# itxtx/normalizing-flows-study

Hardware: AMD Instinct MI355X
Metric: log_prob samples/sec/GPU + test-NLL match; RealNVP d=2 and MAF d=63 (higher is better)
Workload: dtype fp32

## Files before the change

include/nfx.h:

```cpp
#ifndef NFX_H
#define NFX_H

#include <stddef.h>
#include <stdint.h>

#ifdef __cplusplus
extern "C" {
#endif

#define NFX_ABI_VERSION 3

#define NFX_OK 0
#define NFX_EINVAL (-1)
#define NFX_EUNSUPPORTED (-2)
#define NFX_ELAUNCH (-3)

#define NFX_FORWARD 1
#define NFX_INVERSE (-1)

#define NFX_MAF_INVERSE 0
#define NFX_IAF_FORWARD 1
#define NFX_MAF_FORWARD 2
#define NFX_IAF_INVERSE 3

// ... 73 lines not shown
                          int64_t N, int K, float min_bin_width, float min_bin_height, float min_derivative,
                          int inverse, void* stream);

size_t nfx_arqs_packed_floats(int d, int H, int K);
int nfx_arqs_pack(const NfxMlpRaw* made, int d, int H, int K, float* packed, void* stream);
int nfx_arqs(const float* packed, const float* in, float* out, float* log_det, int64_t B, int d,
             int H, int K, float min_bin_width, float min_bin_height, float min_derivative,
             int rescale, double data_min, double data_max, int direction, int accumulate,
             void* stream);

int nfx_base_normal(uint64_t seed, uint64_t* rng_state, float* z, int64_t B, int d, void* stream);

size_t nfx_made_packed_floats(int d, int H);
int nfx_made_pack(const NfxMlpRaw* net, int d, int H, float* packed, void* stream);
int nfx_made_pack_parallel(const NfxMlpRaw* net, int d, int H, float* packed, void* stream);
int nfx_made_pack_sequential(int d, int H, float* packed, void* stream);
int nfx_made_affine(const float* packed, const float* in, float* out, float* log_det,
                    int64_t B, int d, int H, int variant, int accumulate, void* stream);
#define NFX_MADE_SEQ_AUTO 0
#define NFX_MADE_SEQ_SEGMENT 1
#define NFX_MADE_SEQ_WAVE 2
#define NFX_MADE_SEQ_PUSH 3
int nfx_made_seq_policy(int policy);
int nfx_made_affine_logprob(const float* packed, const float* in, float* out, float* log_det,
                            float* logp, double* sums, void* workspace, int64_t B, int d, int H,
                            int variant, int accumulate, void* stream);
int nfx_made_sample_supported(int d, int H, int variant);
int nfx_made_affine_sample(const float* packed, uint64_t seed, uint64_t* rng_state, float* z, float* x,
                           float* log_det, int64_t B, int d, int H, void* stream);

int nfx_made_pack_backward(const NfxMlpRaw* net, int d, int H, float* packed, void* stream);
size_t nfx_made_backward_factor_floats(int64_t B, int d, int H);
int64_t nfx_made_backward_max_batch(int d, int H);
int nfx_made_affine_backward(const float* packed, const float* in, const float* grad_out,
                             const float* grad_log_det, float* grad_in, float* factors, int64_t B,
                             int d, int H, int variant, void* stream);

int nfx_made_seq_backward(const float* packed, const float* in, const float* grad_out,
                          const float* grad_log_det, float* grad_in, float* factors, int64_t B,
                          int d, int H, int variant, void* stream);
int64_t nfx_made_factor_pitch(int64_t B);
size_t nfx_made_param_floats(int d, int H);
size_t nfx_made_wgrad_workspace_bytes(int64_t B, int d, int H);
int nfx_made_backward_weights(const float* factors, int64_t B, int d, int H,
                              const float* const* masks, float* grads, void* workspace,
                              void* stream);
// ... 247 lines not shown
```

normalizing-flows-study_amd/csrc/nfx_made.hip:

```cpp
#include "nfx_made_kernel.h"
#include "nfx_made_wide_kernel.h"
#include <atomic>
#include <cstdlib>

#include "nfx_made_seqs_kernel.h"
#include "nfx_pack.h"

namespace nfx {

__global__ void made_pack_kernel(NfxMlpRaw net, int d, int H, float* packed) {
    const int HT = (H + 31) / 32;
    const MadeLayout L = made_layout(d, HT);
    const int Hp = L.Hp, G1 = 4 * L.NKC;
    for (int i = blockIdx.x * blockDim.x + threadIdx.x; i < L.total; i += gridDim.x * blockDim.x) {
        if (i >= L.s_deg) continue;
        float v = 0.f;
        if (i < L.b1) {
            int t = i - L.w1, rr = t & 3, lane = (t >> 2) & 63, g = (t >> 8) % G1, ht = (t >> 8) / G1;
            int row = 32 * ht + (lane & 31), col = 2 * (4 * g + rr) + (lane >> 5);
            v = (row < H && col < d) ? mlp_weight(net, 0, d, row, col) : 0.f;
        } else if (i < L.w2) {
            int row = acc_vec_row(i - L.b1);
            v = row < H ? mlp_bias(net, 0, row) : 0.f;
        } else if (i < L.b2 || (i >= L.w3 && i < L.b3)) {
            const int layer = i < L.b2 ? 1 : 2;
            const ATileElem e = a_tile_elem(i - (layer == 1 ? L.w2 : L.w3));
            int row = 32 * (e.tile / HT) + e.row, col = 32 * (e.tile % HT) + e.k;
            v = (row < H && col < H) ? mlp_weight(net, layer, H, row, col) : 0.f;
        } else if (i < L.w3 || (i >= L.b3 && i < L.w4)) {
            const int layer = i < L.w3 ? 1 : 2;
            int row = acc_vec_row(i - (layer == 1 ? L.b2 : L.b3));
            v = row < H ? mlp_bias(net, layer, row) : 0.f;
        } else if (i < L.b4) {
            const ATileElem e = a_tile_elem(i - L.w4);
            int jw = e.tile / HT, which = jw & 1, j = jw >> 1;
            int orow = 32 * j + e.row, col = 32 * (e.tile % HT) + e.k;
            v = (orow < d && col < H) ? mlp_weight(net, 3, H, which * d + orow, col) : 0.f;
        } else if (i < L.par_total) {
            int t = i - L.b4, jw = t >> 5, which = jw & 1, j = jw >> 1;
            int orow = 32 * j + acc_vec_row(t & 31);
// ... 37 lines not shown
            if (a < H && net.mask[0]) {
                const float* row = net.mask[0] + (size_t)a * d;
#pragma unroll 4
                for (int j = q; j < d; j += 16) n += row[j] != 0.f ? 1 : 0;
            }
            n += __shfl_xor(n, 1);
            n += __shfl_xor(n, 2);
            n += __shfl_xor(n, 4);
            n += __shfl_xor(n, 8);
            if (q == 0 && a < Hp) deg[a] = a < H ? (net.mask[0] ? n - 1 : 0) : 1000000000;
        }
        __syncthreads();
        for (int a = threadIdx.x; a < Hp; a += kLiveThreads) {
            const int da = deg[a];
            int rank = 0;
            for (int b = 0; b < Hp; ++b) rank += (deg[b] < da || (deg[b] == da && b < a)) ? 1 : 0;
            packed[L.s_deg + a] = (float)da;
            packed[L.s_deg + Hp + rank] = (float)da;
            packed[L.s_deg + 2 * Hp + rank] = (float)a;
        }
    }
    int* nk = reinterpret_cast<int*>(packed);
    for (int i = threadIdx.x; i < 3 * HT + L.NJ; i += kLiveThreads) nk[L.nk1 + i] = 0;
    __shared__ double red[256];
    const int rows[4] = {H, H, H, 2 * d}, cols[4] = {d, H, H, H};
    const double tsafe = block_mlp_tsafe(net, 4, rows, cols, 1.0e37, red);
    if (threadIdx.x == 0) packed[L.tsafe] = (float)fmin(tsafe, 3.0e38);
}

__global__ __launch_bounds__(256) void made_extent_kernel(int d, int H, float* packed) {
    const int HT = (H + 31) / 32;
    const MadeLayout L = made_layout(d, HT);
    int* nk = reinterpret_cast<int*>(packed);
    const int n1 = HT * 4 * L.NKC, n23 = HT * HT * 4, n4 = L.NJ * 2 * HT * 4;
    const int lane = lane_id();
    for (int gi = blockIdx.x * 4 + (threadIdx.x >> 6); gi < n1 + 2 * n23 + n4; gi += gridDim.x * 4) {
        int off, word, ext;
        if (gi < n1) {
            const int ht = gi / (4 * L.NKC), g = gi % (4 * L.NKC);
            off = L.w1 + gi * 256;
            word = L.nk1 + ht;
            ext = g / 4 + 1;
        } else if (gi < n1 + 2 * n23) {
            const int t = (gi - n1) % n23, layer = (gi - n1) / n23;
            off = (layer == 0 ? L.w2 : L.w3) + t * 256;
            word = (layer == 0 ? L.nk2 : L.nk3) + t / (HT * 4);
            ext = (t % (HT * 4)) / 4 + 1;
        } else {
            const int t = gi - n1 - 2 * n23;
            off = L.w4 + t * 256;
            word = L.nk4 + t / (2 * HT * 4);
            ext = (t % (HT * 4)) / 4 + 1;
        }
        const f32x4 v = *reinterpret_cast<const f32x4*>(packed + off + 4 * lane);
        const bool nzl = v[0] != 0.f || v[1] != 0.f || v[2] != 0.f || v[3] != 0.f;
        if (__ballot(nzl) != 0 && lane == 0) atomicMax(&nk[word], ext);
    }
}

template <int HT>
made_seqs_kernel_t made_seqs_pick_ht(int variant, bool logp) {
// ... 60 lines not shown
    return made_pack_seqp(d, H, packed, s);
}
}

extern "C" int nfx_made_pack_parallel(const NfxMlpRaw* net, int d, int H, float* packed, void* stream) {
    if (!net || !packed) return set_error(NFX_EINVAL, "made_pack: null pointer");
    if (d <= 0 || d > 4096 || H <= 0 || H > 256)
        return set_error(NFX_EUNSUPPORTED, "made_pack: d=%d H=%d outside d<=4096, H<=256", d, H);
    if (net->n_layers != 4) return set_error(NFX_EINVAL, "made_pack: MADE has 4 masked layers (got %d)", net->n_layers);
    for (int l = 0; l < 4; ++l)
        if (!net->w[l]) return set_error(NFX_EINVAL, "made_pack: layer %d weight is null", l);
    const int total = (int)nfx_made_packed_floats(d, H);
    int blocks = (total + 255) / 256;
    if (blocks > 2048) blocks = 2048;
    made_pack_kernel<<<blocks, 256, 0, (hipStream_t)stream>>>(*net, d, H, packed);
    int rc = check_launch("made_pack_kernel");
    if (rc) return rc;
    made_live_kernel<<<1, kLiveThreads, 0, (hipStream_t)stream>>>(*net, d, H, packed);
    rc = check_launch("made_live_kernel");
    if (rc) return rc;
    {
        const int HT = (H + 31) / 32;
        const MadeLayout L = made_layout(d, HT);
        const int groups = HT * 4 * L.NKC + 2 * HT * HT * 4 + L.NJ * 2 * HT * 4;
        made_extent_kernel<<<(groups + 3) / 4, 256, 0, (hipStream_t)stream>>>(d, H, packed);
    }
    return check_launch("made_extent_kernel");
}

extern "C" int nfx_made_pack_sequential(int d, int H, float* packed, void* stream) {
    if (!packed) return set_error(NFX_EINVAL, "made_pack_sequential: null pointer");
    if (d <= 0 || d > 4096 || H <= 0 || H > 256)
        return set_error(NFX_EUNSUPPORTED, "made_pack_sequential: d=%d H=%d outside d<=4096, H<=256", d, H);
    return made_pack_seq(d, H, packed, (hipStream_t)stream);
}

extern "C" int nfx_made_pack(const NfxMlpRaw* net, int d, int H, float* packed, void* stream) {
    const int rc = nfx_made_pack_parallel(net, d, H, packed, stream);
    if (rc) return rc;
    return made_pack_seq(d, H, packed, (hipStream_t)stream);
}

namespace nfx {
int made_seqw_launch(const float* packed, const float* in, float* out, float* log_det, int64_t B, int d, int H,
                     int variant, int accumulate, float* logp, double* partials, double* sums, bool fused,
                     int* grid_out, hipStream_t s);
int made_seqp_launch(const float* packed, const float* in, float* out, float* log_det, int64_t B, int d, int H,
                     int variant, int accumulate, float* logp, double* partials, double* sums, bool fused,
                     hipStream_t s);
}

static std::atomic<int>& made_seq_policy() {
    static std::atomic<int> v{[] {
        const char* e = getenv("NFX_MADE_SEQ_POLICY");
        return e ? atoi(e) : NFX_MADE_SEQ_AUTO;
    }()};
    return v;
}

namespace nfx {
int made_seq_policy_get() { return made_seq_policy().load(std::memory_order_relaxed); }
}

static bool tile_path(int d, int HT, int variant) {
    return (variant == NFX_MAF_INVERSE || variant == NFX_IAF_FORWARD) && d > 0 && d <= kTileMaxD && HT >= 1 && HT <= 4;
}

struct TileConfig {
    int nw;
    bool wlds;
    size_t lds;
};
static TileConfig tile_config(const MadeLayout& L, int64_t ntiles, bool fused) {
    int nw = 8;
    if (!fused && ntiles < 4 * (int64_t)num_cus()) nw = (int)((ntiles + num_cus() - 1) / num_cus());
    const size_t wbytes = (size_t)L.par_total * sizeof(float);
    const size_t tiles = nw * 32 * (size_t)kTileStride * sizeof(float);
    const bool wlds = nw == 8 && wbytes + tiles <= kLdsBytes;
    return {nw, wlds, (wlds ? wbytes : 0) + tiles};
}

static int made_launch(const float* packed, const float* in, float* out, float* log_det, int64_t B,
                       int d, int H, int variant, int accumulate, float* logp, double* sums,
                       void* workspace, hipStream_t s) {
// ... 20 lines not shown
                         "made_affine_logprob: fused log_prob needs MAF inverse with d <= %d or H <= 64, "
                         "or IAF inverse with H <= 64", kTileMaxD);
    if (fused && B > 0 && (!logp || !workspace)) return set_error(NFX_EINVAL, "made_affine_logprob: null logp/workspace");
    if (B == 0) return fused ? gauss_finish(reinterpret_cast<double*>(workspace), 0, sums, 0, s) : NFX_OK;
    if (!packed || !in || !out || !log_det) return set_error(NFX_EINVAL, "made_affine: null pointer");
    if (in == out) return set_error(NFX_EINVAL, "made_affine: in and out must not alias");
    double* partials = reinterpret_cast<double*>(workspace);
    if (wide) {
        const int64_t nchunks = (B + 63) / 64;
        const int nw = nchunks < (int64_t)kWideWaves * num_cus() ? 4 : kWideWaves;
        const size_t lds_nw = (size_t)wide_lds(L, HT, nw).total * sizeof(float);
        made_par_kernel_t k = HT == 1 ? made_wide_pick_ht<1>(variant, fused, nw) : made_wide_pick_ht<2>(variant, fused, nw);
        int rc = prepare_lds((const void*)k, lds_nw);
        if (rc) return rc;
        int grid = resident_grid((const void*)k, 64 * nw, lds_nw, (nchunks + nw - 1) / nw);
        if (grid > kMaxPartials) grid = kMaxPartials;
        k<<<grid, 64 * nw, lds_nw, s>>>(packed, in, out, log_det, B, d, accumulate, nchunks, logp, partials,
                                        sums, gauss_const(d));
        return check_launch("made_wide_kernel");
    }
    if (tile_path(d, HT, variant)) {
        const int64_t ntiles = (B + 31) / 32;
        const TileConfig c = tile_config(L, ntiles, fused);
        made_par_kernel_t k = pick_tile(HT, c.wlds, variant, fused);
        if (!k) return set_error(NFX_EUNSUPPORTED, "made_affine: no kernel for H=%d", H);
        int rc = prepare_lds((const void*)k, c.lds);
        if (rc) return rc;
        int grid = resident_grid((const void*)k, 64 * c.nw, c.lds, (ntiles + c.nw - 1) / c.nw);
        if (grid > kMaxPartials) grid = kMaxPartials;
        k<<<grid, 64 * c.nw, c.lds, s>>>(packed, in, out, log_det, B, d, accumulate, ntiles, logp, partials, sums,
                                         gauss_const(d));
        return check_launch("made_tile_kernel");
    }
    if (variant == NFX_MAF_INVERSE || variant == NFX_IAF_FORWARD) {
        const size_t wbytes = (size_t)L.par_total * sizeof(float);
        const size_t stage8 = 8 * (size_t)kStageFloats * sizeof(float);
        const bool wlds = wbytes + stage8 <= kLdsBytes;
        made_par_kernel_t k = pick_par(HT, wlds, variant);
        if (!k) return set_error(NFX_EUNSUPPORTED, "made_affine: no kernel for H=%d", H);
        const int threads = wlds ? 512 : 256;
        const size_t lds = wlds ? wbytes + stage8 : 4 * (size_t)kStageFloats * sizeof(float);
        int rc = prepare_lds((const void*)k, lds);
        if (rc) return rc;
        const int64_t nchunks = (B + 63) / 64;
        const int nw = threads / 64;
        const int grid = resident_grid((const void*)k, threads, lds, (nchunks + nw - 1) / nw);
// ... 18 lines not shown
        const int threads = kSeqsThreads;
        int grid = resident_grid((const void*)k, threads, lds, (B + 4 * kSeqsWaves - 1) / (4 * kSeqsWaves));
        if (grid > kMaxPartials) grid = kMaxPartials;
        k<<<grid, threads, lds, s>>>(packed, in, out, log_det, B, d, H, accumulate, logp, partials, sums,
                                     gauss_const(d));
        return check_launch("made_seqs_kernel");
    }
    made_seq_kernel_t k = pick_seq(HT, variant);
    if (!k) return set_error(NFX_EUNSUPPORTED, "made_affine: no sequential kernel for H=%d", H);
    const size_t lds = 2 * 64 * (size_t)(L.Hp + 4) * sizeof(float);
    int rc = prepare_lds((const void*)k, lds);
    if (rc) return rc;
    const int64_t grid = (B + 63) / 64;
    k<<<(unsigned)grid, 64, lds, s>>>(packed, in, out, log_det, B, d, H, accumulate);
    return check_launch("made_seq_kernel");
}

extern "C" int nfx_made_seq_policy(int policy) {
    if (policy < 0) return made_seq_policy().load();
    if (policy > NFX_MADE_SEQ_PUSH) return set_error(NFX_EINVAL, "made_seq_policy: unknown policy %d", policy);
    return made_seq_policy().exchange(policy);
}

extern "C" int nfx_made_affine(const float* packed, const float* in, float* out, float* log_det,
                               int64_t B, int d, int H, int variant, int accumulate, void* stream) {
    return made_launch(packed, in, out, log_det, B, d, H, variant, accumulate, nullptr, nullptr, nullptr,
                       (hipStream_t)stream);
}

extern "C" int nfx_made_affine_logprob(const float* packed, const float* in, float* out, float* log_det,
                                       float* logp, double* sums, void* workspace, int64_t B, int d,
                                       int H, int variant, int accumulate, void* stream) {
    if (!sums) return set_error(NFX_EINVAL, "made_affine_logprob: null sums");
    return made_launch(packed, in, out, log_det, B, d, H, variant, accumulate, logp, sums, workspace,
                       (hipStream_t)stream);
}

extern "C" int nfx_made_sample_supported(int d, int H, int variant) {
    return (H > 0 && tile_path(d, (H + 31) / 32, variant) && variant == NFX_IAF_FORWARD) ? 1 : 0;
}

extern "C" int nfx_made_affine_sample(const float* packed, uint64_t seed, uint64_t* rng_state, float* z, float* x,
                                      float* log_det, int64_t B, int d, int H, void* stream) {
    if (B < 0 || d <= 0 || H <= 0) return set_error(NFX_EINVAL, "made_affine_sample: bad shape");
    if (!nfx_made_sample_supported(d, H, NFX_IAF_FORWARD))
        return set_error(NFX_EUNSUPPORTED, "made_affine_sample: d=%d H=%d outside the tile kernel (d <= %d, H <= 128)",
// ... 19 lines not shown
```

normalizing-flows-study_amd/csrc/nfx_made_kernel.h:

```cpp
#pragma once
#include "nfx_common.h"
#include "nfx_rng.h"

namespace nfx {

struct MadeLayout {
    int d, HT, Hp, NKC, NJ;
    int w1, b1, w2, b2, w3, b3, w4, b4;
    int par_total;
    int s_w1t, s_b1, s_w2, s_b2, s_w3, s_b3, s_w4, s_b4, s_deg;
    int nk1, nk2, nk3, nk4, tsafe;
    int t4, t3, t2, t1;
    int rimg;
    int sw1, sw4, sb4;
    int ctab;
    int ps, pw4, pw1, pb4, pw23, ptb, ptab;
    int total;
};

__host__ __device__ constexpr int made_up4(int v) { return (v + 3) & ~3; }

__host__ __device__ constexpr int seqs_w4_stride(int Hp) { return 2 * Hp + 4; }
constexpr int kSeqsPadRows = 64;
__host__ __device__ constexpr int seqs_max_chunks(int d, int Hp) { return d / 8 + 2 * Hp + 8; }
constexpr int kSeqpMaxS = 16;
__host__ __device__ constexpr int seqp_slots(int d, int HT) {
    return (HT <= 2 && d <= 64 * kSeqpMaxS) ? (d + 63) / 64 : 0;
}
__host__ __device__ constexpr int seqp_max_chunks(int d, int Hp) { return (d + 63) / 64 + 3 * Hp + 4; }

__host__ __device__ constexpr MadeLayout made_layout(int d, int HT) {
    MadeLayout L{};
    L.d = d;
    L.HT = HT;
    L.Hp = 32 * HT;
    L.NKC = (d + 31) / 32;
    L.NJ = (d + 31) / 32;
    int o = 0;
    L.w1 = o; o += HT * 4 * L.NKC * 256;
// ... 19 lines not shown
    L.nk3 = o; o += HT;
    L.nk4 = o; o += L.NJ;
    L.tsafe = o; o += 1;
    o = made_up4(o);
    L.t4 = o; o += HT * 2 * L.NJ * 1024;
    L.t3 = o; o += HT * HT * 1024;
    L.t2 = o; o += HT * HT * 1024;
    L.t1 = o; o += L.NKC * HT * 1024;
    L.rimg = o; o += HT <= 2 ? 2 * L.Hp * L.Hp + 5 * L.Hp : 0;
    o = made_up4(o);
    const int rows = HT <= 2 ? d + kSeqsPadRows : 0;
    L.sw1 = o; o += made_up4(rows * L.Hp);
    L.sw4 = o; o += made_up4(rows * seqs_w4_stride(L.Hp));
    L.sb4 = o; o += made_up4(2 * rows);
    L.ctab = o; o += HT <= 2 ? 8 * seqs_max_chunks(d, L.Hp) : 0;
    const int PS = seqp_slots(d, HT);
    L.ps = PS;
    L.pw4 = o; o += L.Hp * ((PS + 1) / 2) * 256;
    L.pw1 = o; o += L.Hp * ((PS + 3) / 4) * 256;
    L.pb4 = o; o += PS * 128;
    L.pw23 = o; o += PS ? 2 * L.Hp * L.Hp : 0;
    L.ptb = o; o += PS ? 4 * L.Hp : 0;
    L.ptab = o; o += PS ? 16 * seqp_max_chunks(d, L.Hp) : 0;
    L.total = o;
    return L;
}

constexpr int kStageStride = 33;
constexpr int kTileStride = 65;
constexpr int kStageFloats = 64 * kStageStride;

template <int VAR>
__device__ __forceinline__ float made_affine(float xv, float mu, float al, float& acc) {
#pragma clang fp contract(off)
    if constexpr (VAR == NFX_MAF_INVERSE) {
        const float a = tclamp(al, -3.f, 3.f);
        acc = acc + a;
        const float z = (xv - mu) * exp_fast(-a);
        return nonfinite(z) ? 0.f : z;
    } else {
        const float a = tclamp(al, -2.f, 2.f);
        const float m = tclamp(mu, -10.f, 10.f);
        acc = acc + a;
        const float y = xv * exp_fast(a) + m;
        return nonfinite(y) ? xv : y;
    }
// ... 608 lines not shown
```

normalizing-flows-study_amd/csrc/nfx_tile.h:

```cpp
#pragma once

#include <hip/hip_runtime.h>

namespace nfx {

__host__ __device__ constexpr int crow(int r, int h) { return (r & 3) + 8 * (r >> 2) + 4 * h; }
__host__ __device__ constexpr int creg(int row) { return (row & 3) + 4 * (row >> 3); }
__host__ __device__ constexpr int chalf(int row) { return (row >> 2) & 1; }

struct RowCol {
    int row, col;
};

struct ATileElem {
    int tile, row, k;
};
__host__ __device__ constexpr ATileElem a_tile_elem(int t) {
    const int rr = t & 3, lane = (t >> 2) & 63, rq = (t >> 8) & 3;
    return {t >> 10, lane & 31, crow(4 * rq + rr, lane >> 5)};
}
__host__ __device__ constexpr int a_tile(int ot, int kt, int NK) { return ot * NK + kt; }
__host__ __device__ constexpr int a_quad(int tile, int rq) { return tile * 4 + rq; }
__host__ __device__ constexpr RowCol a_image_elem(int t, int NK) {
    const ATileElem e = a_tile_elem(t);
    return {32 * (e.tile / NK) + e.row, 32 * (e.tile % NK) + e.k};
}

__host__ __device__ constexpr RowCol a1_elem(int t, int KS1) {
    const int lane = t & 63, ks = (t >> 6) % KS1, ht = (t >> 6) / KS1;
    return {32 * ht + (lane & 31), 2 * ks + (lane >> 5)};
}

__host__ __device__ constexpr int acc_vec_row(int t) { return 32 * (t >> 5) + crow(t & 15, (t >> 4) & 1); }
struct VecRow {
    int vec, row;
};
__host__ __device__ constexpr VecRow acc_rows_elem(int t, int HT) {
    return {t / (32 * HT), acc_vec_row(t % (32 * HT))};
}

__host__ __device__ constexpr RowCol acc_dump_elem(int t) { return {crow(t >> 6, (t >> 5) & 1), t & 31}; }
__host__ __device__ constexpr int acc_dump_index(int row, int col) {
    return creg(row) * 64 + chalf(row) * 32 + col;
}
__host__ __device__ constexpr RowCol lane_dump_elem(int t) { return {crow(t & 15, (t >> 9) & 1), (t >> 4) & 31}; }

namespace tile_check {
constexpr bool crow_round_trips() {
    for (int row = 0; row < 32; ++row)
        if (crow(creg(row), chalf(row)) != row) return false;
    for (int r = 0; r < 16; ++r)
        for (int h = 0; h < 2; ++h)
            if (creg(crow(r, h)) != r || chalf(crow(r, h)) != h) return false;
    return true;
}
constexpr bool a_tile_visits_all() {
    bool seen[32 * 32] = {};
    for (int t = 0; t < 1024; ++t) {
        const ATileElem e = a_tile_elem(t);
        if (e.tile != 0 || e.row < 0 || e.row > 31 || e.k < 0 || e.k > 31 || seen[e.row * 32 + e.k]) return false;
        seen[e.row * 32 + e.k] = true;
    }
    return true;
}
constexpr bool a_tile_encode_inverts() {
    for (int t = 0; t < 3 * 1024; ++t) {
        const ATileElem e = a_tile_elem(t);
        const int r = creg(e.k), lane = e.row + 32 * chalf(e.k);
        if ((a_quad(e.tile, r >> 2) * 64 + lane) * 4 + (r & 3) != t) return false;
    }
// ... 42 lines not shown
```

normalizing-flows-study_amd/nfs_amd/_lib.py:

```python
import ctypes
import os
import threading
import types

import torch

_HERE = os.path.dirname(os.path.abspath(__file__))
LIB_PATH = os.environ.get("NFX_LIB", os.path.join(_HERE, "libnfx.so"))

NFX_OK = 0
NFX_EINVAL = -1
NFX_EUNSUPPORTED = -2
NFX_ELAUNCH = -3
NFX_FORWARD = 1
NFX_INVERSE = -1
NFX_MAF_INVERSE = 0
NFX_IAF_FORWARD = 1
NFX_MAF_FORWARD = 2
NFX_IAF_INVERSE = 3
NFX_AFFINE_AUTO = 0
NFX_AFFINE_STREAMING = 1
NFX_AFFINE_SMALL = 2
NFX_MADE_SEQ_AUTO = 0
NFX_MADE_SEQ_SEGMENT = 1
NFX_MADE_SEQ_WAVE = 2
NFX_MADE_SEQ_PUSH = 3
NFX_RESIDUAL_RELU = 0
NFX_RESIDUAL_ELU = 1
NFX_RESIDUAL_LEAKY_RELU = 2
NFX_RESIDUAL_TANH = 3
NFX_NAF_RELU = 0
NFX_NAF_ELU = 1
NFX_NAF_LEAKY_RELU = 2
NFX_NAF_GELU = 3
NFX_NAF_LAYER_NORM = 1


def NFX_NAF_RESIDUAL(l):
    return 2 << l


class NfxLibraryError(RuntimeError):
    pass


class NfxError(RuntimeError):
    pass


# ... 138 lines not shown
    "nfx_naf_backward_workspace_floats": (_sz, [_i64, _int, _int, _vp]),
    "nfx_naf_backward": (_int, [_vp] * 8 + [_i64, _int, _int, _vp, _int, _int, _f, _f, _vp]),
    "nfx_lowrank_supported": (_int, [_i64, _int, _int]),
    "nfx_lowrank_record_floats": (_sz, [_int]),
    "nfx_lowrank_pack_planar": (_int, [_vp, _vp, _vp, _int, _int, _f, _vp, _vp]),
    "nfx_lowrank_pack_radial": (_int, [_vp, _vp, _vp, _int, _int, _f, _vp, _vp]),
    "nfx_lowrank_pack_sylvester": (_int, [_vp, _vp, _vp, _int, _int, _int, _int, _f, _vp, _vp]),
    "nfx_lowrank_stack": (_int, [_vp, _int, _vp, _vp, _vp, _i64, _int, _int, _int, _vp]),
    "nfx_lrbwd_supported": (_int, [_i64, _int, _int, _int]),
    "nfx_lrbwd_max_layers": (_sz, [_int]),
    "nfx_lrbwd_chunk_rows": (_sz, [_int]),
    "nfx_lrbwd_slots": (_sz, [_i64, _int, _int]),
    "nfx_lrbwd_workspace_floats": (_sz, [_i64, _int, _int]),
    "nfx_lrbwd_stack": (_int, [_vp, _int, _vp, _vp, _vp, _vp, _vp, _i64, _int, _int, _vp]),
    "nfx_lrbwd_param_grads": (_int, [_vp, _i64, _int, _int, _int, _int, _vp, _vp, _vp, _vp, _vp, _vp, _int, _int, _vp]),
    "nfx_rqs_unit": (_int, [_vp, _vp, _vp, _vp, _vp, _vp, _i64, _int, _f, _f, _f, _int, _vp]),
    "nfx_rqs_unit_backward": (_int, [_vp, _vp, _vp, _vp, _vp, _vp, _vp, _vp, _vp, _vp, _i64, _int, _f, _f, _f, _int,
                                     _vp]),
    "nfx_made_packed_floats": (_sz, [_int, _int]),
    "nfx_made_pack": (_int, [ctypes.POINTER(NfxMlpRaw), _int, _int, _vp, _vp]),
    "nfx_made_pack_parallel": (_int, [ctypes.POINTER(NfxMlpRaw), _int, _int, _vp, _vp]),
    "nfx_made_pack_sequential": (_int, [_int, _int, _vp, _vp]),
    "nfx_made_seq_policy": (_int, [_int]),
    "nfx_base_normal": (_int, [ctypes.c_uint64, _vp, _vp, _i64, _int, _vp]),
    "nfx_made_sample_supported": (_int, [_int, _int, _int]),
    "nfx_made_affine_sample": (_int, [_vp, ctypes.c_uint64, _vp, _vp, _vp, _vp, _i64, _int, _int, _vp]),
    "nfx_made_affine": (_int, [_vp, _vp, _vp, _vp, _i64, _int, _int, _int, _int, _vp]),
    "nfx_made_affine_logprob": (_int, [_vp, _vp, _vp, _vp, _vp, _vp, _vp, _i64, _int, _int, _int, _int, _vp]),
    "nfx_made_pack_backward": (_int, [ctypes.POINTER(NfxMlpRaw), _int, _int, _vp, _vp]),
    "nfx_made_backward_factor_floats": (_sz, [_i64, _int, _int]),
    "nfx_made_backward_max_batch": (_i64, [_int, _int]),
    "nfx_made_affine_backward": (_int, [_vp, _vp, _vp, _vp, _vp, _vp, _i64, _int, _int, _int, _vp]),
    "nfx_made_seq_backward": (_int, [_vp, _vp, _vp, _vp, _vp, _vp, _i64, _int, _int, _int, _vp]),
    "nfx_made_factor_pitch": (_i64, [_i64]),
    "nfx_made_param_floats": (_sz, [_int, _int]),
    "nfx_made_wgrad_workspace_bytes": (_sz, [_i64, _int, _int]),
    "nfx_made_backward_weights": (_int, [_vp, _i64, _int, _int, ctypes.POINTER(_vp), _vp, _vp, _vp]),
    "nfx_affine_train_pack_floats": (_sz, [_int, _int]),
    "nfx_affine_train_stats_doubles": (_sz, [_int]),
    "nfx_affine_train_grad_doubles": (_sz, [_int, _int]),
    "nfx_affine_train_param_floats": (_sz, [_int, _int]),
    "nfx_affine_train_workspace_bytes": (_sz, [_i64, _int, _int]),
    "nfx_affine_train_pack": (_int, [ctypes.POINTER(NfxMlpRaw), ctypes.POINTER(NfxMlpRaw), _vp, _vp, _vp, _int,
                                     _int, _vp, _vp, _vp]),
    "nfx_affine_train_stats": (_int, [_vp, _vp, _i64, _int, _int, _int, _vp, _vp, _vp]),
    "nfx_affine_train_update_running": (_int, [_vp, _vp, ctypes.POINTER(_vp), ctypes.POINTER(_vp), _int,
# ... 10 lines not shown
    "nfx_affine_train_output": (_int, [_vp, _vp, _vp, _vp, _vp, _i64, _int, _int, _int, _vp]),
    "nfx_affine_eval_stats": (_int, [ctypes.POINTER(_vp), ctypes.POINTER(_vp), _int, _vp, _vp, _vp]),
    "nfx_spline_backward_packed_floats": (_sz, [_int, _int, _int]),
    "nfx_spline_backward_param_floats": (_sz, [_int, _int, _int]),
    "nfx_spline_backward_workspace_bytes": (_sz, [_i64, _int, _int, _int]),
    "nfx_spline_pack_backward": (_int, [ctypes.POINTER(NfxMlpRaw), _vp, _int, _int, _int, _vp, _vp]),
    "nfx_spline_coupling_backward": (_int, [_vp, _vp, _vp, _vp, _vp, _vp, _vp, _vp, _i64, _int, _int, _int, _int,
                                            _f, _f, _f, _f, _int, _vp]),
    "nfx_gauss_workspace_bytes": (_sz, [_i64]),
    "nfx_gauss_workspace_init": (_int, [_vp, _vp]),
    "nfx_gauss_logprob": (_int, [_vp, _vp, _vp, _vp, _vp, _i64, _int, _vp]),
    "nfx_gauss_logprob_backward": (_int, [_vp, _vp, _vp, _vp, _i64, _int, _vp]),
    "nfx_flowbn_workspace_bytes": (_sz, [_i64, _int]),
    "nfx_flowbn_apply": (_int, [_vp, _vp, _vp, _vp, _vp, _vp, _vp, _f, _i64, _int, _int, _vp]),
    "nfx_flowbn_moments": (_int, [_vp, _i64, _int, _vp, _vp, _vp]),
    "nfx_flowbn_update_running": (_int, [_vp, _vp, _vp, ctypes.c_double, _int, _vp]),
    "nfx_flowbn_backward": (_int, [_vp, _vp, _vp, _vp, _vp, _vp, _vp, _vp, _f, _vp, _vp, _i64, _int, _int,
                                   _vp, _vp]),
}

EXPORTED_SYMBOLS = tuple(_SIGNATURES)

_VALUE_RETURNING = frozenset((
    "nfx_abi_version", "nfx_affine_kernel_policy", "nfx_made_seq_policy", "nfx_affine_chain_supported",
    "nfx_spline_chain_supported", "nfx_cnf_supported", "nfx_cnf_backward_supported",
    "nfx_made_sample_supported", "nfx_residual_supported", "nfx_residual_backward_supported",
    "nfx_naf_supported", "nfx_naf_backward_supported",
    "nfx_lowrank_supported", "nfx_lrbwd_supported"))


_as_pointer = _vp.from_param


class DevicePtr:

    @staticmethod
    def from_param(v):
        if v is None or type(v) is int:
            return _as_pointer(v)
        return _as_pointer(v.data_ptr())


def _raise_on_status(rc, fn, args):
    if rc != NFX_OK:
        raise NfxError(f"{fn.__name__} failed (rc={rc}): {lib().nfx_last_error().decode(errors='replace')}")
    return rc

# ... 115 lines not shown
```

Baseline: 1.678 billion.

## Add 16x16x4 MFMA tile kernel for small MADE with finer sparsity skipping

Adds a MADE forward/log-prob kernel built on 16x16x4 fp32 MFMA instead of 32x32x2. It uses a new packed 16-row weight layout with per-block extent words, so masked-zero blocks can be skipped at finer granularity. In auto mode it replaces the existing tile path only for H<=64 (HT==2), d>32, MAF inverse, with an 8-wave LDS config, and an environment/ABI policy knob can force either path. It adds packing cost and packed-buffer size, and uses an LDS-staged x tile with a swizzled layout.

```diff
diff --git a/include/nfx.h b/include/nfx.h
--- a/include/nfx.h
+++ b/include/nfx.h
@@ -119,6 +119,10 @@
 #define NFX_MADE_SEQ_WAVE 2
 #define NFX_MADE_SEQ_PUSH 3
 int nfx_made_seq_policy(int policy);
+#define NFX_MADE_TILE_AUTO 0
+#define NFX_MADE_TILE_32 1
+#define NFX_MADE_TILE_16 2
+int nfx_made_tile_policy(int policy);
 int nfx_made_affine_logprob(const float* packed, const float* in, float* out, float* log_det,
                             float* logp, double* sums, void* workspace, int64_t B, int d, int H,
                             int variant, int accumulate, void* stream);
diff --git a/normalizing-flows-study_amd/csrc/nfx_made.hip b/normalizing-flows-study_amd/csrc/nfx_made.hip
--- a/normalizing-flows-study_amd/csrc/nfx_made.hip
+++ b/normalizing-flows-study_amd/csrc/nfx_made.hip
@@ -1,4 +1,5 @@
 #include "nfx_made_kernel.h"
+#include "nfx_made_tile16_kernel.h"
 #include "nfx_made_wide_kernel.h"
 #include <atomic>
 #include <cstdlib>
@@ -7,15 +8,45 @@
 #include "nfx_pack.h"
 
 namespace nfx {
+
+__device__ float made_pack16_value(const NfxMlpRaw& net, int d, int H, const MadeLayout& L, int i) {
+    const int NT = L.NT, NK = L.NK16;
+    if (i < L.qb1) {
+        const A16Elem e = a16_elem(i - L.q1);
+        const int row = 16 * (e.blk / NK) + unit16(e.row), col = 16 * (e.blk % NK) + e.kpos;
+        return (row < H && col < d) ? mlp_weight(net, 0, d, row, col) : 0.f;
+    }
+    if (i < L.q4) {
+        const int layer = i < L.q2 ? 0 : (i < L.q3 ? 1 : 2);
+        const int bbase = layer == 0 ? L.qb1 : (layer == 1 ? L.qb2 : L.qb3);
+        if (i >= bbase) {
+            const int t = i - bbase, row = 16 * (t >> 4) + unit16(t & 15);
+            return row < H ? mlp_bias(net, layer, row) : 0.f;
+        }
+        const A16Elem e = a16_elem(i - (layer == 1 ? L.q2 : L.q3));
+        const int row = 16 * (e.blk / NT) + unit16(e.row), col = 16 * (e.blk % NT) + unit16(chain16_row(e.kpos));
+        return (row < H && col < H) ? mlp_weight(net, layer, H, row, col) : 0.f;
+    }
+    if (i < L.qb4) {
+        const A16Elem e = a16_elem(i - L.q4);
+        const int jw = e.blk / NT, orow = 16 * (jw >> 1) + out16_dim(e.row);
+        const int col = 16 * (e.blk % NT) + unit16(chain16_row(e.kpos));
+        return (orow < d && col < H) ? mlp_weight(net, 3, H, (jw & 1) * d + orow, col) : 0.f;
+    }
+    const int t = i - L.qb4, jw = t >> 4, orow = 16 * (jw >> 1) + out16_dim(t & 15);
+    return orow < d ? mlp_bias(net, 3, (jw & 1) * d + orow) : 0.f;
+}
 
 __global__ void made_pack_kernel(NfxMlpRaw net, int d, int H, float* packed) {
     const int HT = (H + 31) / 32;
     const MadeLayout L = made_layout(d, HT);
     const int Hp = L.Hp, G1 = 4 * L.NKC;
     for (int i = blockIdx.x * blockDim.x + threadIdx.x; i < L.total; i += gridDim.x * blockDim.x) {
-        if (i >= L.s_deg) continue;
+        if (i >= L.s_deg && (i < L.q1 || i >= L.e1)) continue;
         float v = 0.f;
-        if (i < L.b1) {
+        if (i >= L.q1) {
+            v = made_pack16_value(net, d, H, L, i);
+        } else if (i < L.b1) {
             int t = i - L.w1, rr = t & 3, lane = (t >> 2) & 63, g = (t >> 8) % G1, ht = (t >> 8) / G1;
             int row = 32 * ht + (lane & 31), col = 2 * (4 * g + rr) + (lane >> 5);
             v = (row < H && col < d) ? mlp_weight(net, 0, d, row, col) : 0.f;
@@ -99,6 +130,7 @@
     }
     int* nk = reinterpret_cast<int*>(packed);
     for (int i = threadIdx.x; i < 3 * HT + L.NJ; i += kLiveThreads) nk[L.nk1 + i] = 0;
+    for (int i = threadIdx.x; i < 3 * L.NT + L.NK16; i += kLiveThreads) nk[L.e1 + i] = 0;
     __shared__ double red[256];
     const int rows[4] = {H, H, H, 2 * d}, cols[4] = {d, H, H, H};
     const double tsafe = block_mlp_tsafe(net, 4, rows, cols, 1.0e37, red);
@@ -110,10 +142,29 @@
     const MadeLayout L = made_layout(d, HT);
     int* nk = reinterpret_cast<int*>(packed);
     const int n1 = HT * 4 * L.NKC, n23 = HT * HT * 4, n4 = L.NJ * 2 * HT * 4;
+    const int m1 = L.NT * L.NK16, m23 = L.NT * L.NT, m4 = L.NK16 * 2 * L.NT;
+    const int n32 = n1 + 2 * n23 + n4;
     const int lane = lane_id();
-    for (int gi = blockIdx.x * 4 + (threadIdx.x >> 6); gi < n1 + 2 * n23 + n4; gi += gridDim.x * 4) {
+    for (int gi = blockIdx.x * 4 + (threadIdx.x >> 6); gi < n32 + m1 + 2 * m23 + m4; gi += gridDim.x * 4) {
         int off, word, ext;
-        if (gi < n1) {
+        if (gi >= n32) {
+            const int b = gi - n32;
+            if (b < m1) {
+                off = L.q1 + b * 256;
+                word = L.e1 + b / L.NK16;
+                ext = b % L.NK16 + 1;
+            } else if (b < m1 + 2 * m23) {
+                const int t = (b - m1) % m23, layer = (b - m1) / m23;
+                off = (layer == 0 ? L.q2 : L.q3) + t * 256;
+                word = (layer == 0 ? L.e2 : L.e3) + t / L.NT;
+                ext = t % L.NT + 1;
+            } else {
+                const int t = b - m1 - 2 * m23;
+                off = L.q4 + t * 256;
+                word = L.e4 + t / (2 * L.NT);
+                ext = t % L.NT + 1;
+            }
+        } else if (gi < n1) {
             const int ht = gi / (4 * L.NKC), g = gi % (4 * L.NKC);
             off = L.w1 + gi * 256;
             word = L.nk1 + ht;
@@ -220,7 +271,8 @@
     {
         const int HT = (H + 31) / 32;
         const MadeLayout L = made_layout(d, HT);
-        const int groups = HT * 4 * L.NKC + 2 * HT * HT * 4 + L.NJ * 2 * HT * 4;
+        const int groups = HT * 4 * L.NKC + 2 * HT * HT * 4 + L.NJ * 2 * HT * 4 + L.NT * L.NK16 +
+                           2 * L.NT * L.NT + L.NK16 * 2 * L.NT;
         made_extent_kernel<<<(groups + 3) / 4, 256, 0, (hipStream_t)stream>>>(d, H, packed);
     }
     return check_launch("made_extent_kernel");
@@ -258,6 +310,15 @@
 
 namespace nfx {
 int made_seq_policy_get() { return made_seq_policy().load(std::memory_order_relaxed); }
+}
+
+static std::atomic<int>& made_tile_policy() {
+    static std::atomic<int> v{[] {
+        const char* e = getenv("NFX_MADE_TILE_POLICY");
+        const int p = e ? atoi(e) : NFX_MADE_TILE_AUTO;
+        return p >= NFX_MADE_TILE_AUTO && p <= NFX_MADE_TILE_16 ? p : NFX_MADE_TILE_AUTO;
+    }()};
+    return v;
 }
 
 static bool tile_path(int d, int HT, int variant) {
@@ -324,6 +385,20 @@
     if (tile_path(d, HT, variant)) {
         const int64_t ntiles = (B + 31) / 32;
         const TileConfig c = tile_config(L, ntiles, fused);
+        const int tile_pol = made_tile_policy().load(std::memory_order_relaxed);
+        made_par_kernel_t k16 = tile_pol == NFX_MADE_TILE_32 ? nullptr : made_tile16_pick(L.NT ? HT : 0, variant, fused);
+        if (tile_pol == NFX_MADE_TILE_AUTO && !(c.nw == 8 && c.wlds && HT == 2 && d > 32 && variant == NFX_MAF_INVERSE))
+            k16 = nullptr;
+        if (k16) {
+            const size_t lds16 = ((size_t)L.q_total + 8 * 32 * (size_t)kTile16Stride) * sizeof(float);
+            int rc = prepare_lds((const void*)k16, lds16);
+            if (rc) return rc;
+            int grid = resident_grid((const void*)k16, 512, lds16, (ntiles + 7) / 8);
+            if (grid > kMaxPartials) grid = kMaxPartials;
+            k16<<<grid, 512, lds16, s>>>(packed, in, out, log_det, B, d, accumulate, ntiles, logp, partials, sums,
+                                         gauss_const(d));
+            return check_launch("made_tile16_kernel");
+        }
         made_par_kernel_t k = pick_tile(HT, c.wlds, variant, fused);
         if (!k) return set_error(NFX_EUNSUPPORTED, "made_affine: no kernel for H=%d", H);
         int rc = prepare_lds((const void*)k, c.lds);
@@ -388,6 +463,12 @@
     return made_seq_policy().exchange(policy);
 }
 
+extern "C" int nfx_made_tile_policy(int policy) {
+    if (policy < 0) return made_tile_policy().load();
+    if (policy > NFX_MADE_TILE_16) return set_error(NFX_EINVAL, "made_tile_policy: unknown policy %d", policy);
+    return made_tile_policy().exchange(policy);
+}
+
 extern "C" int nfx_made_affine(const float* packed, const float* in, float* out, float* log_det,
                                int64_t B, int d, int H, int variant, int accumulate, void* stream) {
     return made_launch(packed, in, out, log_det, B, d, H, variant, accumulate, nullptr, nullptr, nullptr,
diff --git a/normalizing-flows-study_amd/csrc/nfx_made_kernel.h b/normalizing-flows-study_amd/csrc/nfx_made_kernel.h
--- a/normalizing-flows-study_amd/csrc/nfx_made_kernel.h
+++ b/normalizing-flows-study_amd/csrc/nfx_made_kernel.h
@@ -15,6 +15,7 @@
     int sw1, sw4, sb4;
     int ctab;
     int ps, pw4, pw1, pb4, pw23, ptb, ptab;
+    int NT, NK16, q1, qb1, q2, qb2, q3, qb3, q4, qb4, q_total, e1, e2, e3, e4;
     int total;
 };
 
@@ -80,6 +81,25 @@
     L.pw23 = o; o += PS ? 2 * L.Hp * L.Hp : 0;
     L.ptb = o; o += PS ? 4 * L.Hp : 0;
     L.ptab = o; o += PS ? 16 * seqp_max_chunks(d, L.Hp) : 0;
+    const bool t16 = HT <= 2 && d <= 64;
+    const int NT = t16 ? 2 * HT : 0, NK16 = t16 ? (d + 15) / 16 : 0;
+    L.NT = NT;
+    L.NK16 = NK16;
+    o = made_up4(o);
+    L.q1 = o; o += NT * NK16 * 256;
+    L.qb1 = o; o += NT * 16;
+    L.q2 = o; o += NT * NT * 256;
+    L.qb2 = o; o += NT * 16;
+    L.q3 = o; o += NT * NT * 256;
+    L.qb3 = o; o += NT * 16;
+    L.q4 = o; o += NK16 * 2 * NT * 256;
+    L.qb4 = o; o += NK16 * 2 * 16;
+    L.q_total = o - L.q1;
+    L.e1 = o; o += NT;
+    L.e2 = o; o += NT;
+    L.e3 = o; o += NT;
+    L.e4 = o; o += NK16;
+    o = made_up4(o);
     L.total = o;
     return L;
 }
diff --git a/normalizing-flows-study_amd/csrc/nfx_made_tile16.hip b/normalizing-flows-study_amd/csrc/nfx_made_tile16.hip
--- /dev/null
+++ b/normalizing-flows-study_amd/csrc/nfx_made_tile16.hip
@@ -0,0 +1,17 @@
+#include "nfx_made_tile16_kernel.h"
+
+namespace nfx {
+
+template <int HT>
+static made_par_kernel_t tile16_var(int variant, bool logp) {
+    if (variant != NFX_MAF_INVERSE) return made_tile16_kernel<HT, NFX_IAF_FORWARD, false>;
+    return logp ? made_tile16_kernel<HT, NFX_MAF_INVERSE, true> : made_tile16_kernel<HT, NFX_MAF_INVERSE, false>;
+}
+
+made_par_kernel_t made_tile16_pick(int HT, int variant, bool logp) {
+    if (HT == 1) return tile16_var<1>(variant, logp);
+    if (HT == 2) return tile16_var<2>(variant, logp);
+    return nullptr;
+}
+
+}
diff --git a/normalizing-flows-study_amd/csrc/nfx_made_tile16_kernel.h b/normalizing-flows-study_amd/csrc/nfx_made_tile16_kernel.h
--- /dev/null
+++ b/normalizing-flows-study_amd/csrc/nfx_made_tile16_kernel.h
@@ -0,0 +1,282 @@
+#pragma once
+#include "nfx_made_kernel.h"
+
+namespace nfx {
+
+__device__ __forceinline__ f32x4 mfma16(float a, float b, f32x4 c) {
+    return __builtin_amdgcn_mfma_f32_16x16x4f32(a, b, c, 0, 0, 0);
+}
+
+template <int VAR>
+__device__ __forceinline__ float made_affine16(float xv, float mu, float al, float& a) {
+    float zero = 0.f;
+    const float z = made_affine<VAR>(xv, mu, al, zero);
+    a = zero;
+    return z;
+}
+
+__device__ __forceinline__ f32x4 lds_quad(const float* p) { return *reinterpret_cast<const f32x4*>(p); }
+
+template <int NTO, int KT>
+__device__ __forceinline__ void layer16(const float* __restrict__ W, int woff, int kimg, int boff, const int (&n)[NTO],
+                                        const f32x4 (&hin)[KT][2], f32x4 (&hout)[NTO][2]) {
+    const int lane = lane_id(), g = lane >> 4;
+    f32x4 w[2][KT], b[2][2];
+    b[0][0] = lds_quad(W + boff + 4 * g);
+    b[0][1] = lds_quad(W + boff + opaque_zero() + 4 * g);
+#pragma unroll
+    for (int kt = 0; kt < KT; ++kt) w[0][kt] = lds_quad(W + woff + (kt * 64 + lane) * 4);
+#pragma unroll
+    for (int T = 0; T < NTO; ++T) {
+        if (T + 1 < NTO) {
+            b[(T + 1) & 1][0] = lds_quad(W + boff + (T + 1) * 16 + 4 * g);
+            b[(T + 1) & 1][1] = lds_quad(W + boff + opaque_zero() + (T + 1) * 16 + 4 * g);
+#pragma unroll
+            for (int kt = 0; kt < KT; ++kt) w[(T + 1) & 1][kt] = lds_quad(W + woff + (((T + 1) * kimg + kt) * 64 + lane) * 4);
+        }
+        f32x4 a0 = b[T & 1][0], a1 = b[T & 1][1];
+#pragma unroll
+        for (int kt = 0; kt < KT; ++kt) {
+            if (kt < n[T]) {
+#pragma unroll
+                for (int rr = 0; rr < 4; ++rr) {
+                    a0 = mfma16(w[T & 1][kt][rr], hin[kt][0][rr], a0);
+                    a1 = mfma16(w[T & 1][kt][rr], hin[kt][1][rr], a1);
+                }
+            }
+        }
+#pragma unroll
+        for (int r = 0; r < 4; ++r) {
+            a0[r] = trelu(a0[r]);
+            a1[r] = trelu(a1[r]);
+        }
+        hout[T][0] = a0;
+        hout[T][1] = a1;
+    }
+}
+
+__device__ __forceinline__ float groups_up(float v) {
+    auto r = __builtin_amdgcn_permlane16_swap(__float_as_uint(v), __float_as_uint(v), false, false);
+    return __uint_as_float(r[0]);
+}
+__device__ __forceinline__ float groups_down(float v) {
+    auto r = __builtin_amdgcn_permlane16_swap(__float_as_uint(v), __float_as_uint(v), false, false);
+    return __uint_as_float(r[1]);
+}
+
+template <int HT, int VAR, bool LOGP>
+__global__ __launch_bounds__(512) void made_tile16_kernel(
+    const float* __restrict__ packed, const float* __restrict__ in, float* __restrict__ out,
+    float* __restrict__ logdet, int64_t B, int d, int accumulate, int64_t ntiles,
+    float* __restrict__ logp, double* __restrict__ partials, double* __restrict__ sums, float cgauss) {
+    constexpr int NT = 2 * HT;
+    constexpr int S = kTile16Stride;
+    const MadeLayout L = made_layout(d, HT);
+    const int NK = L.NK16;
+    extern __shared__ f32x4 lds4[];
+    float* lds = reinterpret_cast<float*>(lds4);
+    const int wave = __builtin_amdgcn_readfirstlane(threadIdx.x >> 6);
+    {
+        const f32x4* src = reinterpret_cast<const f32x4*>(packed + L.q1);
+        for (int i = threadIdx.x; i < L.q_total / 4; i += 512) lds4[i] = src[i];
+    }
+    float* xt = lds + L.q_total + wave * 32 * S;
+    __syncthreads();
+    const int lane = lane_id(), col = lane & 31, s16 = lane & 15, g = lane >> 4;
+    const int64_t nwaves = (int64_t)gridDim.x * 8;
+    const int voff = lane < d ? lane * 4 : (1 << 30);
+    const int rowb = d * 4;
+    const int xcol = x16_col(lane);
+    int xb[4], eb[4];
+#pragma unroll
+    for (int r = 0; r < 4; ++r) {
+        xb[r] = s16 * S + x16_col(4 * r + g);
+        eb[r] = s16 * S + x16_col(out16_dim(crow16(r, g)));
+    }
+    const int* nkp = reinterpret_cast<const int*>(packed);
+    int e1[NT], e2[NT], e3[NT];
+#pragma unroll
+    for (int i = 0; i < NT; ++i) {
+        e1[i] = nkp[L.e1 + i];
+        e2[i] = nkp[L.e2 + i];
+        e3[i] = nkp[L.e3 + i];
+    }
+    int e4[4];
+#pragma unroll
+    for (int j = 0; j < 4; ++j) {
+        const int n16 = j < NK ? nkp[L.e4 + j] : 0, n32 = j < NK ? nkp[L.nk4 + (j >> 1)] : 0;
+        e4[j] = n16 > 0 ? n16 : (n32 > 0 ? 1 : 0);
+    }
+    const float tsafe = packed[L.tsafe];
+
+    int64_t t = (int64_t)blockIdx.x * 8 + wave;
+    double lpacc = 0.0;
+    float pf[32];
+    float ldpf = 0.f;
+    {
+        if (accumulate && t < ntiles && lane < 32 && t * 32 + col < B) ldpf = logdet[t * 32 + col];
+        const int64_t rows = t < ntiles ? (B - t * 32 < 32 ? B - t * 32 : 32) : 0;
+        const auto rs = __builtin_amdgcn_make_buffer_rsrc(const_cast<float*>(in) + (t < ntiles ? t * 32 * d : 0), 0,
+                                                          (int)(rows * rowb), 0x00020000);
+#pragma unroll
+        for (int r = 0; r < 32; ++r)
+            pf[r] = __uint_as_float(__builtin_amdgcn_raw_buffer_load_b32(rs, voff, r * rowb, 0));
+    }
+    for (; t < ntiles; t += nwaves) {
+        const int64_t base = t * 32;
+        const int rows = (int)(B - base < 32 ? B - base : 32);
+        const float* W = lds + opaque_zero();
+        float xmax = 0.f;
+#pragma unroll
+        for (int r = 0; r < 32; ++r) {
+            xt[r * S + xcol] = pf[r];
+            xmax = tmax(xmax, fabsf(pf[r]));
+        }
+        const bool dense = __builtin_amdgcn_ballot_w64(!(xmax <= tsafe)) != 0;
+        wave_lds_sync();
+
+        const float ldin = ldpf;
+        {
+            const int64_t tn = t + nwaves;
+            ldpf = (accumulate && tn < ntiles && lane < 32 && tn * 32 + col < B) ? logdet[tn * 32 + col] : 0.f;
+            const int64_t rn = tn < ntiles ? (B - tn * 32 < 32 ? B - tn * 32 : 32) : 0;
+            const auto rs = __builtin_amdgcn_make_buffer_rsrc(const_cast<float*>(in) + (tn < ntiles ? tn * 32 * d : 0), 0,
+                                                              (int)(rn * rowb), 0x00020000);
+#pragma unroll
+            for (int r = 0; r < 32; ++r)
+                pf[r] = __uint_as_float(__builtin_amdgcn_raw_buffer_load_b32(rs, voff, r * rowb, 0));
+        }
+
+        f32x4 x0[4][2];
+#pragma unroll
+        for (int kt = 0; kt < 4; ++kt)
+#pragma unroll
+            for (int c = 0; c < 2; ++c)
+#pragma unroll
+                for (int r = 0; r < 4; ++r) x0[kt][c][r] = xt[xb[r] + c * 16 * S + 16 * kt];
+        int n1[NT], n2[NT], n3[NT];
+#pragma unroll
+        for (int T = 0; T < NT; ++T) {
+            n1[T] = dense ? NK : e1[T];
+            n2[T] = dense ? NT : e2[T];
+            n3[T] = dense ? NT : e3[T];
+        }
+        f32x4 h1[NT][2], h2[NT][2];
+        layer16<NT, 4>(W, 0, NK, L.qb1 - L.q1, n1, x0, h1);
+        layer16<NT, NT>(W, L.q2 - L.q1, NT, L.qb2 - L.q1, n2, h1, h2);
+        layer16<NT, NT>(W, L.q3 - L.q1, NT, L.qb3 - L.q1, n3, h2, h1);
+
+        float acc[2] = {0.f, 0.f}, accup1 = 0.f;
+        f32x4 w4[2][2][NT], b4[2][2][2];
+        const int w4off = L.q4 - L.q1, b4off = L.qb4 - L.q1;
+#pragma unroll
+        for (int which = 0; which < 2; ++which) {
+            b4[0][which][0] = lds_quad(W + b4off + which * 16 + 4 * g);
+            b4[0][which][1] = lds_quad(W + b4off + opaque_zero() + which * 16 + 4 * g);
+#pragma unroll
+            for (int kt = 0; kt < NT; ++kt) w4[0][which][kt] = lds_quad(W + w4off + ((which * NT + kt) * 64 + lane) * 4);
+        }
+#pragma unroll
+        for (int j = 0; j < 4; ++j) {
+            if (j < NK) {
+                if (j + 1 < NK) {
+#pragma unroll
+                    for (int which = 0; which < 2; ++which) {
+                        b4[(j + 1) & 1][which][0] = lds_quad(W + b4off + ((j + 1) * 2 + which) * 16 + 4 * g);
+                        b4[(j + 1) & 1][which][1] = lds_quad(W + b4off + opaque_zero() + ((j + 1) * 2 + which) * 16 + 4 * g);
+#pragma unroll
+                        for (int kt = 0; kt < NT; ++kt)
+                            w4[(j + 1) & 1][which][kt] =
+                                lds_quad(W + w4off + ((((j + 1) * 2 + which) * NT + kt) * 64 + lane) * 4);
+                    }
+                }
+                f32x4 mu[2] = {b4[j & 1][0][0], b4[j & 1][0][1]}, al[2] = {b4[j & 1][1][0], b4[j & 1][1][1]};
+                const int n4 = dense ? NT : e4[j];
+#pragma unroll
+                for (int kt = 0; kt < NT; ++kt) {
+                    if (kt < n4) {
+#pragma unroll
+                        for (int rr = 0; rr < 4; ++rr) {
+                            mu[0] = mfma16(w4[j & 1][0][kt][rr], h1[kt][0][rr], mu[0]);
+                            mu[1] = mfma16(w4[j & 1][0][kt][rr], h1[kt][1][rr], mu[1]);
+                            al[0] = mfma16(w4[j & 1][1][kt][rr], h1[kt][0][rr], al[0]);
+                            al[1] = mfma16(w4[j & 1][1][kt][rr], h1[kt][1][rr], al[1]);
+                        }
+                    }
+                }
+#pragma unroll
+                for (int c = 0; c < 2; ++c) {
+                    float a[4];
+#pragma unroll
+                    for (int r = 0; r < 4; ++r) {
+                        float* p = xt + eb[r] + c * 16 * S + 16 * j;
+                        *p = made_affine16<VAR>(*p, mu[c][r], al[c][r], a[r]);
+                    }
+                    float v = acc[c];
+#pragma unroll
+                    for (int r = 0; r < 4; ++r) v = v + a[r];
+                    float u = groups_up(v);
+#pragma unroll
+                    for (int r = 0; r < 4; ++r) u = u + a[r];
+                    if (c == 1) accup1 = u;
+                    acc[c] = groups_down(u);
+                }
+            }
+        }
+        const float half = (g & 1) ? accup1 : acc[0];
+        const float ssum = halves_sum(half, half);
+        wave_lds_sync();
+        float zsq = 0.f;
+        if constexpr (LOGP) {
+            if (lane < 32) {
+#pragma unroll
+                for (int q = 0; q < 16; ++q) {
+                    if (4 * q < d) {
+                        const f32x4 v4 = *reinterpret_cast<const f32x4*>(xt + col * S + 4 * q);
+#pragma unroll
+                        for (int e = 0; e < 4; ++e) {
+                            if (4 * q + e < d) {
+                                const float v = v4[x16_col(4 * q + e) & 3];
+                                zsq = (4 * q + e == 0) ? gauss_sq0(v) : gauss_sq(zsq, v);
+                            }
+                        }
+                    }
+                }
+            }
+        }
+        {
+            const auto rs = __builtin_amdgcn_make_buffer_rsrc(out + base * d, 0, rows * rowb, 0x00020000);
+#pragma unroll
+            for (int r = 0; r < 32; ++r)
+                __builtin_amdgcn_raw_buffer_store_b32(__float_as_uint(xt[r * S + xcol]), rs, voff, r * rowb, 0);
+        }
+        if (lane < 32 && col < rows) {
+            float ldv;
+            if constexpr (VAR == NFX_MAF_INVERSE) {
+                ldv = -ssum;
+                if (nonfinite(ldv)) ldv = 0.f;
+                ldv = tclamp(ldv, -100.f, 100.f);
+            } else {
+                ldv = ssum;
+                if (nonfinite(ldv)) ldv = 0.f;
+                ldv = tclamp(ldv, -50.f, 50.f);
+            }
+            const int64_t so = base + col;
+            const float ldt = accumulate ? ldin + ldv : ldv;
+            logdet[so] = ldt;
+            if constexpr (LOGP) {
+                const float lp = gauss_lp(zsq, cgauss, ldt);
+                logp[so] = lp;
+                lpacc += (double)lp;
+            }
+        }
+        wave_lds_sync();
+    }
+    if constexpr (LOGP) {
+        logp_commit<512>(lpacc, partials, sums, B);
+    }
+}
+
+made_par_kernel_t made_tile16_pick(int HT, int variant, bool logp);
+
+}
diff --git a/normalizing-flows-study_amd/csrc/nfx_tile.h b/normalizing-flows-study_amd/csrc/nfx_tile.h
--- a/normalizing-flows-study_amd/csrc/nfx_tile.h
+++ b/normalizing-flows-study_amd/csrc/nfx_tile.h
@@ -45,7 +45,76 @@
 }
 __host__ __device__ constexpr RowCol lane_dump_elem(int t) { return {crow(t & 15, (t >> 9) & 1), (t >> 4) & 31}; }
 
+__host__ __device__ constexpr int crow16(int r, int g) { return 4 * g + r; }
+__host__ __device__ constexpr int creg16(int row) { return row & 3; }
+__host__ __device__ constexpr int cgrp16(int row) { return row >> 2; }
+__host__ __device__ constexpr int chain16_pos(int row) { return 4 * creg16(row) + cgrp16(row); }
+__host__ __device__ constexpr int chain16_row(int p) { return crow16(p >> 2, p & 3); }
+__host__ __device__ constexpr int unit16(int row) { return crow(chain16_pos(row) >> 1, chain16_pos(row) & 1); }
+__host__ __device__ constexpr int blk16(int g) { return ((g & 1) << 1) | (g >> 1); }
+__host__ __device__ constexpr int out16_dim(int row) { return 4 * blk16(cgrp16(row)) + creg16(row); }
+__host__ __device__ constexpr int x16_col(int D) { return D ^ ((D >> 2) & 3); }
+constexpr int kTile16Stride = 68;
+
+struct A16Elem {
+    int blk, row, kpos;
+};
+__host__ __device__ constexpr A16Elem a16_elem(int t) {
+    const int rr = t & 3, lane = (t >> 2) & 63;
+    return {t >> 8, lane & 15, 4 * rr + (lane >> 4)};
+}
+
 namespace tile_check {
+constexpr bool chain16_matches_32() {
+    for (int q = 0; q < 32; ++q) {
+        const int old_unit = crow(q >> 1, q & 1);
+        const int kt = q >> 4, p = q & 15;
+        if (16 * kt + unit16(crow16(p >> 2, p & 3)) != old_unit) return false;
+        if (chain16_pos(chain16_row(p)) != p) return false;
+    }
+    return true;
+}
+constexpr bool rows16_are_bijections() {
+    bool u[16] = {}, o[16] = {}, c[64] = {};
+    for (int row = 0; row < 16; ++row) {
+        if (crow16(creg16(row), cgrp16(row)) != row) return false;
+        if (u[unit16(row)] || o[out16_dim(row)]) return false;
+        u[unit16(row)] = o[out16_dim(row)] = true;
+    }
+    for (int D = 0; D < 64; ++D) {
+        if (x16_col(D) < 0 || x16_col(D) > 63 || (x16_col(D) >> 2) != (D >> 2) || c[x16_col(D)]) return false;
+        c[x16_col(D)] = true;
+    }
+    return true;
+}
+constexpr bool a16_visits_all() {
+    bool seen[16 * 16] = {};
+    for (int t = 0; t < 256; ++t) {
+        const A16Elem e = a16_elem(t);
+        if (e.blk != 0 || seen[e.row * 16 + e.kpos]) return false;
+        seen[e.row * 16 + e.kpos] = true;
+    }
+    return a16_elem(256 + 5).blk == 1;
+}
+constexpr bool x16_banks_two_lanes() {
+    for (int r = 0; r < 4; ++r) {
+        int b1[32] = {}, b4[32] = {};
+        for (int l = 0; l < 64; ++l) {
+            const int s = l & 15, g = l >> 4;
+            ++b1[(s * kTile16Stride + x16_col(4 * r + g)) & 31];
+            ++b4[(s * kTile16Stride + x16_col(out16_dim(crow16(r, g)))) & 31];
+        }
+        for (int b = 0; b < 32; ++b)
+            if (b1[b] != 2 || b4[b] != 2) return false;
+    }
+    return true;
+}
+static_assert(chain16_matches_32(), "the 16x16x4 chain consumes the 32x32x2 form's unit at every position");
+static_assert(rows16_are_bijections(), "unit16, out16_dim and x16_col are bijections");
+static_assert(a16_visits_all(), "16-row A-operand decode is a bijection onto the block");
+static_assert(x16_banks_two_lanes(), "x tile: two lanes per LDS bank for layer 1 and the epilogue");
+static_assert(kTile16Stride % 4 == 0, "16-byte row reads of the x tile");
+
 constexpr bool crow_round_trips() {
     for (int row = 0; row < 32; ++row)
         if (crow(creg(row), chalf(row)) != row) return false;
diff --git a/normalizing-flows-study_amd/nfs_amd/_lib.py b/normalizing-flows-study_amd/nfs_amd/_lib.py
--- a/normalizing-flows-study_amd/nfs_amd/_lib.py
+++ b/normalizing-flows-study_amd/nfs_amd/_lib.py
@@ -25,6 +25,9 @@
 NFX_MADE_SEQ_SEGMENT = 1
 NFX_MADE_SEQ_WAVE = 2
 NFX_MADE_SEQ_PUSH = 3
+NFX_MADE_TILE_AUTO = 0
+NFX_MADE_TILE_32 = 1
+NFX_MADE_TILE_16 = 2
 NFX_RESIDUAL_RELU = 0
 NFX_RESIDUAL_ELU = 1
 NFX_RESIDUAL_LEAKY_RELU = 2
@@ -209,6 +212,7 @@
     "nfx_made_pack_parallel": (_int, [ctypes.POINTER(NfxMlpRaw), _int, _int, _vp, _vp]),
     "nfx_made_pack_sequential": (_int, [_int, _int, _vp, _vp]),
     "nfx_made_seq_policy": (_int, [_int]),
+    "nfx_made_tile_policy": (_int, [_int]),
     "nfx_base_normal": (_int, [ctypes.c_uint64, _vp, _vp, _i64, _int, _vp]),
     "nfx_made_sample_supported": (_int, [_int, _int, _int]),
     "nfx_made_affine_sample": (_int, [_vp, ctypes.c_uint64, _vp, _vp, _vp, _vp, _i64, _int, _int, _vp]),
@@ -265,7 +269,8 @@
 EXPORTED_SYMBOLS = tuple(_SIGNATURES)
 
 _VALUE_RETURNING = frozenset((
-    "nfx_abi_version", "nfx_affine_kernel_policy", "nfx_made_seq_policy", "nfx_affine_chain_supported",
+    "nfx_abi_version", "nfx_affine_kernel_policy", "nfx_made_seq_policy", "nfx_made_tile_policy",
+    "nfx_affine_chain_supported",
     "nfx_spline_chain_supported", "nfx_cnf_supported", "nfx_cnf_backward_supported",
     "nfx_made_sample_supported", "nfx_residual_supported", "nfx_residual_backward_supported",
     "nfx_naf_supported", "nfx_naf_backward_supported",
```

Result: no change. 1.677 billion (-0.1%).
